# vbronetskyi/nclt-slam-project

Measured on AMD Instinct MI355X. Metric: relocalization frames/sec @640x480, 10k-landmark DB; Hamming-match HBM GB/s, higher is better.
Workload: dtype u8; 1 GPU; 640x480 BGR frames, 10000-record landmark DB (640000 descriptors, rows=fixed64), global relocalization tick per frame: ORB(500) + whole-DB mutual Hamming scan + top-25 PnP-RANSAC(200); frames resident in HBM, every frame's 96-byte result record written to pinned host memory by the tick's last kernel; distinct_frames=32, preroll_steps=20, streams=4, records=10000, descriptors=640000, parallelism=frames sharded across ranks, database replicated, no collective

## Files before the change

### nclt-slam-project_amd/csrc/reloc_match.hip

```cpp
#include <stdlib.h>
#include <type_traits>
#include <utility>

#include "reloc_internal.h"

typedef uint32_t u32;

__device__ __forceinline__ u32 bcnt_acc(u32 x, u32 acc)
{
    u32 r;
    asm("v_bcnt_u32_b32 %0, %1, %2" : "=v"(r) : "v"(x), "v"(acc));
    return r;
}
__device__ __forceinline__ u32 min_u16(u32 a, u32 b)
{
    u32 r;
    asm("v_min_u16 %0, %1, %2" : "=v"(r) : "v"(a), "v"(b));
    return r;
}
template <u32 IDX>
__device__ __forceinline__ u32 key_fma(u32 d, u32 c128)
{
    u32 r;
    asm("v_fmaak_f32 %0, %1, %2, %3" : "=v"(r) : "v"(d), "v"(c128), "n"(IDX));
    return r;
}
__device__ __forceinline__ u32 ham8(const u32 q[8], const uint4 a, const uint4 b, u32 init)
{
    u32 acc = init;
    acc = bcnt_acc(q[0] ^ a.x, acc);
    acc = bcnt_acc(q[1] ^ a.y, acc);
    acc = bcnt_acc(q[2] ^ a.z, acc);
    acc = bcnt_acc(q[3] ^ a.w, acc);
    acc = bcnt_acc(q[4] ^ b.x, acc);
    acc = bcnt_acc(q[5] ^ b.y, acc);
    acc = bcnt_acc(q[6] ^ b.z, acc);
    acc = bcnt_acc(q[7] ^ b.w, acc);
    return acc;
}

__device__ __forceinline__ void ham8x2(const u32 q0[8], const u32 q1[8], const uint4 a, const uint4 b, u32 init0, u32 init1,
                                       u32 &d0, u32 &d1)
{
    const u32 w[8] = {a.x, a.y, a.z, a.w, b.x, b.y, b.z, b.w};
    u32 acc0 = init0, acc1 = init1;
#pragma unroll
    for (int k = 0; k < 8; ++k) {
        const u32 x0 = q0[k] ^ w[k], x1 = q1[k] ^ w[k];
        acc0 = bcnt_acc(x0, acc0);
        acc1 = bcnt_acc(x1, acc1);
    }
    d0 = acc0;
    d1 = acc1;
}

template <int NC>
__device__ __forceinline__ void ham8_cols(const u32 (&q)[NC][8], const u32 (&w)[8], u32 (&h)[NC])
{
#pragma unroll
    for (int k = 0; k < 8; ++k)
#pragma unroll
        for (int j = 0; j < NC; ++j) {
            u32 x;
            asm volatile("v_xor_b32 %0, %1, %2" : "=v"(x) : "s"(w[k]), "v"(q[j][k]));
            if (k == 0) asm volatile("v_bcnt_u32_b32 %0, %1, 0" : "=v"(h[j]) : "v"(x));
            else asm volatile("v_bcnt_u32_b32 %0, %1, %0" : "+v"(h[j]) : "v"(x));
        }
}

__device__ __forceinline__ void srow_landed(u32 first_dword) { asm volatile("" ::"s"(first_dword)); }

__device__ __forceinline__ u32 umin(u32 a, u32 b) { return a < b ? a : b; }
__device__ __forceinline__ double uniform_f64(double v)
{
    return __hiloint2double(__builtin_amdgcn_readfirstlane(__double2hiint(v)), __builtin_amdgcn_readfirstlane(__double2loint(v)));
}
__device__ __forceinline__ u32 umax(u32 a, u32 b) { return a > b ? a : b; }

template <int K>
__device__ __forceinline__ u32 bfly(u32 a, u32 b, int lane)
{
    if constexpr (K == 32) {
        auto r = __builtin_amdgcn_permlane32_swap(a, b, false, false);
        return umin(r[0], r[1]);
    } else if constexpr (K == 16) {
        auto r = __builtin_amdgcn_permlane16_swap(a, b, false, false);
        return umin(r[0], r[1]);
    } else {
        const bool hi = lane & K;
        const u32 mine = hi ? b : a;
        const u32 theirs = hi ? a : b;
        return umin(mine, dpp_xor<K>(theirs));
    }
}

template <int K>
__device__ __forceinline__ u32 bfly_dpp(u32 a, u32 b)
{
    static_assert(K == 4 || K == 8, "bank-maskable lane bits only");
    u32 r;
    if constexpr (K == 4)
        asm("s_nop 1\n\tv_min_u32_dpp %0, %1, %1 row_shl:4 row_mask:0xf bank_mask:0x5\n\t"
            "v_min_u32_dpp %0, %2, %2 row_shr:4 row_mask:0xf bank_mask:0xa" : "=&v"(r) : "v"(a), "v"(b));
    else
        asm("s_nop 1\n\tv_min_u32_dpp %0, %1, %1 row_ror:8 row_mask:0xf bank_mask:0x3\n\t"
            "v_min_u32_dpp %0, %2, %2 row_ror:8 row_mask:0xf bank_mask:0xc" : "=&v"(r) : "v"(a), "v"(b));
    return r;
}
__device__ __forceinline__ u32 allmin_quad(u32 x)
{
    asm("s_nop 1\n\tv_min_u32_dpp %0, %0, %0 quad_perm:[1,0,3,2] row_mask:0xf bank_mask:0xf\n\t"
        "s_nop 1\n\tv_min_u32_dpp %0, %0, %0 quad_perm:[2,3,0,1] row_mask:0xf bank_mask:0xf" : "+v"(x));
    return x;
}

__device__ __forceinline__ u32 row_entry(u32 best, u32 lane)
{
    u32 v;
    asm("v_lshl_or_b32 %0, %1, 6, %2" : "=v"(v) : "v"(best), "v"(lane));
    return v;
}
__device__ __forceinline__ u32 row_key(u32 m, u32 colbase) { return ((m << 3) & 0xFFFF0000u) | ((m & 0x1FFu) | colbase); }
__device__ __forceinline__ u32 col_key(u32 k16, int tc)
{
    u32 key = k16 << 9;
    const u32 row = (k16 >> 3) & 15u;
    asm("v_add_u32_sdwa %0, %1, %2 dst_sel:WORD_0 dst_unused:UNUSED_PRESERVE src0_sel:DWORD src1_sel:DWORD"
        : "+v"(key) : "s"(tc), "v"(row));
    return key;
}

template <class F, int... I>
__device__ __forceinline__ void static_for_impl(F &&f, std::integer_sequence<int, I...>) { (f(std::integral_constant<int, I>{}), ...); }
template <int N, class F>
__device__ __forceinline__ void static_for(F &&f) { static_for_impl(f, std::make_integer_sequence<int, N>{}); }

template <int NJ>
__device__ __forceinline__ void scan_chunk(const uint4 *__restrict__ rec, int n, int tc, int nr, const u32 (&q)[NJ][8],
                                           u32 colbase, u32 *rowkey, u32 *colbest, bool single_cb, int lane)
{
    u32 cb16[NJ];
    const u32 c128 = 0x43000000u;
    constexpr int R = 16, LOG_R = 4;
    u32 stk[LOG_R + 1];
    auto bitrev = [](int i) { int r = 0; for (int b = 0; b < LOG_R; ++b) r |= ((i >> b) & 1) << (LOG_R - 1 - b); return r; };
    auto row_of = [&](int i) { return min(tc + bitrev(i), n - 1); };
    uint4 a = rec[2 * row_of(0)], b = rec[2 * row_of(0) + 1];
    static_for<R>([&](auto ic_) {
        constexpr int i = decltype(ic_)::value;
        constexpr int t = [](int v) { int r = 0; for (int bb = 0; bb < LOG_R; ++bb) r |= ((v >> bb) & 1) << (LOG_R - 1 - bb); return r; }(i);
        srow_landed(a.x);
        uint4 na, nb;
        if (i + 1 < R) { na = rec[2 * row_of(i + 1)]; nb = rec[2 * row_of(i + 1) + 1]; }
        __builtin_amdgcn_sched_barrier(0);
        u32 v = 0xFFFFFFFFu;
        if (t == 0 || t < nr) {
            u32 best = 0;
            const u32 w[8] = {a.x, a.y, a.z, a.w, b.x, b.y, b.z, b.w};
            u32 h[NJ];
            ham8_cols<NJ>(q, w, h);
            static_for<NJ / 2>([&](auto jc_) {
                constexpr int j = 2 * decltype(jc_)::value;
                const u32 k0 = key_fma<t * 8 + j>(h[j], c128), k1 = key_fma<t * 8 + j + 1>(h[j + 1], c128);
                cb16[j] = t == 0 ? k0 : min_u16(cb16[j], k0);
                cb16[j + 1] = t == 0 ? k1 : min_u16(cb16[j + 1], k1);
                best = j == 0 ? min_u16(k0, k1) : min_u16(best, min_u16(k0, k1));
            });
            v = row_entry(best, (u32)lane);
        }
        if constexpr ((i & 1) == 0) stk[0] = v;
        else {
            v = bfly_dpp<4>(stk[0], v);
            if constexpr ((i & 2) == 0) stk[1] = v;
            else {
                v = bfly_dpp<8>(stk[1], v);
                if constexpr ((i & 4) == 0) stk[2] = v;
                else {
                    v = bfly<16>(stk[2], v, lane);
                    if constexpr ((i & 8) == 0) stk[3] = v;
                    else stk[4] = bfly<32>(stk[3], v, lane);
                }
            }
        }
        __builtin_amdgcn_sched_barrier(0);
        if (i + 1 < R) { a = na; b = nb; }
    });
    const u32 m = allmin_quad(stk[LOG_R]);
    const int row_in_chunk = ((lane >> 2) & 1) * 8 + ((lane >> 3) & 1) * 4 + ((lane >> 4) & 1) * 2 + (lane >> 5);
    const bool writer = (lane & 3) == 0;
    const int row = tc + row_in_chunk;
    if (writer && row_in_chunk < nr) {
        if (single_cb) rowkey[row] = row_key(m, 0);
        else atomicMin(&rowkey[row], row_key(m, colbase));
    }
    u32 ck[NJ];
#pragma unroll
    for (int j = 0; j < NJ; ++j) ck[j] = col_key(cb16[j], tc);
    __builtin_amdgcn_sched_barrier(0);
#pragma unroll
    for (int j = 0; j < NJ; ++j) atomicMin(&colbest[colbase + j * 64 + lane], ck[j]);
}

struct WaveBinding {
    bool bound;
    int my_cb;
    int chunk0, chunk_step;
};
template <int NW>
__device__ __forceinline__ WaveBinding bind_wave(int wave, int ncb)
{
    const bool bound = (NW % ncb) == 0;
    return {bound, bound ? wave % ncb : 0, bound ? wave / ncb : wave, bound ? NW / ncb : NW};
}

template <int NJ, int NW>
__device__ __forceinline__ void db_emit_body(
    u32 *lds, int C, const uint4 *__restrict__ db, const int64_t *__restrict__ off, const int32_t *__restrict__ rec_ids,
    const int32_t *__restrict__ n_ids_p, int n_ids_max, const uint4 *__restrict__ cur, int max_rows,
    int32_t *__restrict__ m_qidx, int32_t *__restrict__ m_tidx, int32_t *__restrict__ m_dist, int32_t *__restrict__ m_n,
    int emit_stride, const float *__restrict__ g_pts3d, const float *__restrict__ g_xy, float *__restrict__ g_obj,
    float *__restrict__ g_img)
{
    constexpr int CB = 64 * NJ;
    const int tid = threadIdx.x, lane = tid & 63;
    const int wave = __builtin_amdgcn_readfirstlane(tid >> 6);
    const int n_ids = n_ids_p ? min(*n_ids_p, n_ids_max) : n_ids_max;
    const int ncb = max((C + CB - 1) / CB, 1);
    u32 *colbest = lds;
    u32 *rowkey = colbest + ncb * CB;
    u32 *wsum = rowkey + max_rows;
    static_assert(NW == 1 || NW == 2 || NW == 4 || NW == 8, "wsum holds one word per wave");

    u32 q[NJ][8];
    auto load_q = [&](int colbase) {
#pragma unroll
        for (int j = 0; j < NJ; ++j) {
            const int col = min(colbase + j * 64 + lane, max(C - 1, 0));
            const uint4 a = cur[2 * col], b = cur[2 * col + 1];
            q[j][0] = a.x; q[j][1] = a.y; q[j][2] = a.z; q[j][3] = a.w;
            q[j][4] = b.x; q[j][5] = b.y; q[j][6] = b.z; q[j][7] = b.w;
        }
    };
    const WaveBinding wb = bind_wave<NW>(wave, ncb);
    if (wb.bound) load_q(wb.my_cb * CB);
    for (int it = blockIdx.x; it < n_ids; it += gridDim.x) {
        const int r = rec_ids ? rec_ids[it] : it;
        const int64_t row0 = off[r];
        const int n = (int)(off[r + 1] - row0);
        const uint4 *rec = db + 2 * row0;
        for (int i = tid; i < ncb * CB; i += 64 * NW) colbest[i] = 0xFFFFFFFFu;
        for (int i = tid; i < n; i += 64 * NW) rowkey[i] = 0xFFFFFFFFu;
        __syncthreads();
        if (n > 0 && C > 0) {
            for (int cb = wb.bound ? wb.my_cb : 0; cb < (wb.bound ? wb.my_cb + 1 : ncb); ++cb) {
                if (!wb.bound) load_q(cb * CB);
                const int per = n / wb.chunk_step, extra = n % wb.chunk_step;
                int tc = wb.chunk0 * per + min(wb.chunk0, extra);
                const int tend = tc + per + (wb.chunk0 < extra ? 1 : 0);
#pragma nounroll
                for (; tc < tend; tc += 16)
                    scan_chunk<NJ>(rec, n, tc, min(16, tend - tc), q, (u32)(cb * CB), rowkey, colbest, ncb == 1, lane);
            }
        }
        __syncthreads();
        u32 base = 0;
        for (int rb = 0; rb < n; rb += 64 * NW) {
            const int row = rb + tid;
            bool mutual = false;
            u32 key = 0;
            if (row < n && C > 0) {
                key = rowkey[row];
                const u32 col = key & 0xFFFFu;
                mutual = (colbest[col] & 0xFFFFu) == (u32)row;
            }
            const unsigned long long bal = __ballot(mutual);
            if (lane == 0) wsum[wave] = (u32)__popcll(bal);
            __syncthreads();
            u32 before = base;
            for (int w = 0; w < wave; ++w) before += wsum[w];
            u32 total = 0;
            for (int w = 0; w < NW; ++w) total += wsum[w];
            if (mutual) {
                const u32 pos = before + (u32)__popcll(bal & ((1ull << lane) - 1ull));
                const int64_t o = (int64_t)it * emit_stride + pos;
                m_qidx[o] = row;
                m_tidx[o] = (int32_t)(key & 0xFFFFu);
                m_dist[o] = (int32_t)(key >> 16);
                if (g_obj) {
                    const float *p3 = g_pts3d + 3 * (row0 + row), *p2 = g_xy + 2 * (size_t)(key & 0xFFFFu);
                    float *po = g_obj + 3 * o, *pi = g_img + 2 * o;
                    po[0] = p3[0]; po[1] = p3[1]; po[2] = p3[2];
                    pi[0] = p2[0]; pi[1] = p2[1];
                }
            }
            base += total;
            __syncthreads();
        }
        if (tid == 0 && m_n) m_n[it] = (int32_t)base;
    }
}

constexpr int TICKET_STRIDE = 32;
constexpr int SCAN_TICKET_WORDS = (RELOC_BATCH_MAX * 8 + 1) * TICKET_STRIDE;
template <int NJ>
__device__ __forceinline__ void db_count_body(
    u32 *lds, int C, const uint4 *__restrict__ db, const int64_t *__restrict__ off, const int32_t *__restrict__ rec_ids,
    const int32_t *__restrict__ n_ids_p, int n_ids_max, const uint4 *__restrict__ cur, int max_rows,
    int32_t *__restrict__ counts, const ScanMask &mask, u32 *ticket, int quota, int n_bounded, int col_words,
    u32 *ticket_pool = nullptr, int pool_frames = 1, int block = -1, int n_blocks = -1)
{
    if (!ticket_pool) ticket_pool = ticket;
    if (block < 0) { block = blockIdx.x; n_blocks = gridDim.x; }
    constexpr int CB = 64 * NJ, NW = 4;
    const int tid = threadIdx.x, lane = tid & 63;
    const int wave = __builtin_amdgcn_readfirstlane(tid >> 6);
    const int n_ids = n_ids_p ? min(*n_ids_p, n_ids_max) : n_ids_max;
    const int ncb = max((C + CB - 1) / CB, 1);
    const bool dbl = 2 * ncb * CB <= col_words;
    u32 *colbuf = lds;
    u32 *rowkey = colbuf + col_words;
    u32 *wsum = rowkey + max_rows;

    u32 q[NJ][8];
    auto load_q = [&](int colbase) {
#pragma unroll
        for (int j = 0; j < NJ; ++j) {
            const int col = min(colbase + j * 64 + lane, max(C - 1, 0));
            const uint4 a = cur[2 * col], b = cur[2 * col + 1];
            q[j][0] = a.x; q[j][1] = a.y; q[j][2] = a.z; q[j][3] = a.w;
            q[j][4] = b.x; q[j][5] = b.y; q[j][6] = b.z; q[j][7] = b.w;
        }
    };
    const WaveBinding wb = bind_wave<NW>(wave, ncb);
    const bool stand_down = mask.skip_if && *mask.skip_if != 0;
    if (wb.bound && !stand_down) load_q(wb.my_cb * CB);
    double hc = 1.0, hs = 0.0, cos_tol = 0.0;
    if (mask.xyh) {
        cur_heading_q(mask.q, hc, hs);
        cos_tol = mask.cos_tol;
        hc = uniform_f64(hc); hs = uniform_f64(hs); cos_tol = uniform_f64(cos_tol);
    }
    int shard = 0, dry = 0;
    if (ticket) {
        u32 x;
        asm volatile("s_getreg_b32 %0, hwreg(HW_REG_XCC_ID, 0, 4)" : "=s"(x));
        shard = (int)(x & 7u);
    }
    auto draw = [&]() -> u32 { return atomicAdd(&ticket[shard * TICKET_STRIDE], 1u); };
    auto settle = [&](u32 t) -> int {
        for (;;) {
            const long long rec_i = (long long)n_blocks + (long long)shard + 8ll * (long long)t;
            if (rec_i < n_ids) return (int)rec_i;
            if (++dry >= 8) return n_ids;
            shard = (shard + 1) & 7;
            t = draw();
        }
    };
    int it = stand_down ? n_ids : block;
    int left = (quota > 0 && block < n_bounded) ? quota : 0x7fffffff;
    const bool dealer = tid == 64 * (NW - 1);
    const int buf_words = ncb * CB;
    for (int i = tid; i < buf_words; i += 64 * NW) colbuf[i] = 0xFFFFFFFFu;
    if (tid == 0) wsum[0] = wsum[1] = 0;
    __syncthreads();
    int p = 0;
    while (it < n_ids) {
        u32 *colbest = colbuf + (dbl ? p * buf_words : 0);
        const int r = rec_ids ? rec_ids[it] : it;
        const bool scored = !(mask.xyh && !heading_ok(mask.xyh + 4 * (int64_t)r, hc, hs, cos_tol));
        const int64_t row0 = off[r];
        const int n_rec = scored ? (int)(off[r + 1] - row0) : 0;
        const int n = C > 0 ? n_rec : 0;
        const uint4 *rec = db + 2 * row0;
        left -= max(n_rec, 1);
        u32 next_ticket = 0;
        if (ticket && dealer && left > 0) next_ticket = draw();
        if (n > 0) {
            if (ncb > 1) {
                for (int i = tid; i < n; i += 64 * NW) rowkey[i] = 0xFFFFFFFFu;
                __syncthreads();
            }
            for (int cb = wb.bound ? wb.my_cb : 0; cb < (wb.bound ? wb.my_cb + 1 : ncb); ++cb) {
                if (!wb.bound) load_q(cb * CB);
                const int per = n / wb.chunk_step, extra = n % wb.chunk_step;
                int tc = wb.chunk0 * per + min(wb.chunk0, extra);
                const int tend = tc + per + (wb.chunk0 < extra ? 1 : 0);
#pragma nounroll
                for (; tc < tend; tc += 16)
                    scan_chunk<NJ>(rec, n, tc, min(16, tend - tc), q, (u32)(cb * CB), rowkey, colbest, ncb == 1, lane);
            }
        }
        if (dbl) {
            u32 *other = colbuf + (p ^ 1) * buf_words;
            for (int base = 0; base + 128 * wave < buf_words; base += 128 * NW) {
                other[base + 2 * tid] = 0xFFFFFFFFu;
                other[base + 2 * tid + 1] = 0xFFFFFFFFu;
            }
        }
        __syncthreads();
        for (int rb = 0; rb + 64 * wave < n; rb += 64 * NW) {
            const int row = rb + tid;
            if (row < n) {
                const u32 col = rowkey[row] & 0xFFFFu;
                const unsigned long long mutual = __builtin_amdgcn_ballot_w64((colbest[col] & 0xFFFFu) == (u32)row);
                if (lane == 0 && mutual) atomicAdd(&wsum[p], (u32)__popcll(mutual));
            }
        }
        if (dealer) wsum[8] = ticket ? (left > 0 ? (u32)settle(next_ticket) : (u32)n_ids) : (u32)(it + n_blocks);
        __syncthreads();
        if (tid == 0) {
            counts[r] = (int32_t)wsum[p];
            wsum[p] = 0;
        }
        it = __builtin_amdgcn_readfirstlane((int)wsum[8]);
        if (dbl) p ^= 1;
        else {
            for (int i = tid; i < ncb * CB; i += 64 * NW) colbuf[i] = 0xFFFFFFFFu;
            __syncthreads();
        }
    }
    if (ticket && tid == 0) {
        const int words = pool_frames * 8;
        if (atomicAdd(&ticket_pool[words * TICKET_STRIDE], 1u) == gridDim.x - 1) {
            for (int x = 0; x <= words; ++x)
                __hip_atomic_store(&ticket_pool[x * TICKET_STRIDE], 0u, __ATOMIC_RELAXED, __HIP_MEMORY_SCOPE_AGENT);
        }
    }
}

template <int NJ>
__global__ __launch_bounds__(256, 4) RELOC_SCAN_VGPR_ATTR void k_db_scan(
    const uint4 *__restrict__ db, const int64_t *__restrict__ off, const int32_t *__restrict__ rec_ids,
    const int32_t *__restrict__ n_ids_p, int n_ids_max, const uint4 *__restrict__ cur,
    const int32_t *__restrict__ n_cur_p, int n_cur_max, int max_rows, int32_t *__restrict__ counts, ScanMask mask, u32 *ticket,
    int quota, int n_bounded, int col_words)
{
    extern __shared__ u32 lds[];
    const int C = n_cur_p ? min(*n_cur_p, n_cur_max) : n_cur_max;
    db_count_body<NJ>(lds, C, db, off, rec_ids, n_ids_p, n_ids_max, cur, max_rows, counts, mask, ticket, quota, n_bounded, col_words);
}

template <int NJ, int NW>
__global__ __launch_bounds__(64 * NW, 16 / NW) RELOC_SCAN_VGPR_ATTR void k_db_scan_emit(
    const uint4 *__restrict__ db, const int64_t *__restrict__ off, const int32_t *__restrict__ rec_ids,
    const int32_t *__restrict__ n_ids_p, int n_ids_max, const uint4 *__restrict__ cur,
    const int32_t *__restrict__ n_cur_p, int n_cur_max, int max_rows, int32_t *__restrict__ m_qidx,
    int32_t *__restrict__ m_tidx, int32_t *__restrict__ m_dist, int32_t *__restrict__ m_n, int emit_stride,
    const float *__restrict__ g_pts3d, const float *__restrict__ g_xy, float *__restrict__ g_obj, float *__restrict__ g_img)
{
    extern __shared__ u32 lds[];
    RELOC_SMALL_KERNEL_PRIO();
    const int C = n_cur_p ? min(*n_cur_p, n_cur_max) : n_cur_max;
    db_emit_body<NJ, NW>(lds, C, db, off, rec_ids, n_ids_p, n_ids_max, cur, max_rows, m_qidx, m_tidx, m_dist, m_n, emit_stride, g_pts3d,
                         g_xy, g_obj, g_img);
}

struct EmitFrame {
    const int32_t *rec_ids, *n_ids_p; const uint4 *cur; const int32_t *n_cur_p;
    int32_t *m_qidx, *m_tidx, *m_dist, *m_n; const float *g_xy; float *g_obj, *g_img;
};
struct EmitBatch { EmitFrame f[RELOC_BATCH_MAX]; };
static EmitFrame emit_frame(const reloc_ctx *c)
{
    EmitFrame F;
    const TickState &t = c->tick;
    const OrbFrame &o = c->orb.buf;
    F.rec_ids = t.cand_ids; F.n_ids_p = t.cand_n; F.cur = (const uint4 *)o.f_desc; F.n_cur_p = o.f_count;
    F.m_qidx = t.m_qidx; F.m_tidx = t.m_tidx; F.m_dist = t.m_dist; F.m_n = t.m_n; F.g_xy = o.f_xy; F.g_obj = t.p_obj; F.g_img = t.p_img;
    return F;
}

__global__ __launch_bounds__(256, 4) RELOC_SCAN_VGPR_ATTR void k_db_scan_emit_batch(const uint4 *__restrict__ db, const int64_t *__restrict__ off, int n_ids_max,
                                                          int n_cur_max, int max_rows, int emit_stride, const float *__restrict__ g_pts3d,
                                                          EmitBatch bt)
{
    extern __shared__ u32 lds[];
    RELOC_SMALL_KERNEL_PRIO();
    const EmitFrame &F = bt.f[blockIdx.y];
    const int C = F.n_cur_p ? min(*F.n_cur_p, n_cur_max) : n_cur_max;
    db_emit_body<8, 4>(lds, C, db, off, F.rec_ids, F.n_ids_p, n_ids_max, F.cur, max_rows, F.m_qidx, F.m_tidx, F.m_dist, F.m_n, emit_stride,
                       g_pts3d, F.g_xy, F.g_obj, F.g_img);
}

static int scan_lds_bytes(const char *who, int col_words, int max_rows, size_t &lds)
{
    lds = (size_t)(col_words + max_rows + 16) * 4;
    if (lds > 160 * 1024) { reloc_set_error("%s: LDS demand %zu bytes", who, lds); return RELOC_E_CAPACITY; }
    return RELOC_OK;
}

struct ScanBatch {
    int n;
    const uint4 *cur[RELOC_BATCH_MAX];
    const int32_t *n_cur[RELOC_BATCH_MAX];
    int32_t *counts[RELOC_BATCH_MAX];
    const int32_t *skip_if[RELOC_BATCH_MAX];
    double q[RELOC_BATCH_MAX][4];
    const double *xyh;
    double cos_tol;
};

__global__ __launch_bounds__(256, 4) RELOC_SCAN_VGPR_ATTR void k_db_scan_batch(const uint4 *__restrict__ db, const int64_t *__restrict__ off, int n_ids,
                                                          int n_cur_max, int max_rows, ScanBatch bt, u32 *ticket_pool, int quota, int n_bounded, int col_words)
{
    extern __shared__ u32 lds[];
    const int f = blockIdx.x % bt.n;
    ScanMask mask;
    mask.xyh = bt.xyh;
    for (int k = 0; k < 4; ++k) mask.q[k] = bt.q[f][k];
    mask.cos_tol = bt.cos_tol;
    mask.skip_if = bt.skip_if[f];
    const int C = bt.n_cur[f] ? min(*bt.n_cur[f], n_cur_max) : n_cur_max;
    db_count_body<8>(lds, C, db, off, nullptr, nullptr, n_ids, bt.cur[f], max_rows, bt.counts[f], mask, ticket_pool + f * 8 * TICKET_STRIDE, quota,
                     n_bounded, col_words, ticket_pool, bt.n, (int)(blockIdx.x / bt.n), (int)((gridDim.x + bt.n - 1 - f) / bt.n));
}

__device__ __forceinline__ u32 max_u16(u32 a, u32 b)
{
    u32 r;
    asm("v_max_u16 %0, %1, %2" : "=v"(r) : "v"(a), "v"(b));
    return r;
}

template <bool TICK>
__device__ __forceinline__ void db_ratio_body(const uint4 *__restrict__ db, const int64_t *__restrict__ off, int n_rec,
                                              const uint4 *__restrict__ cur, int C, double ratio, int32_t *__restrict__ counts,
                                              const ScanMask &mask, int min_rows, int block, int n_blocks)
{
    __shared__ u32 s_part[4][512];
    __shared__ int s_cnt[4];
    const int tid = threadIdx.x, lane = tid & 63;
    const int wave = __builtin_amdgcn_readfirstlane(tid >> 6);
    const int ncb = max((C + 511) >> 9, 1);
    double hc = 1.0, hs = 0.0, cos_tol = 0.0;
    if constexpr (TICK) {
        if (mask.skip_if && *mask.skip_if != 0) return;
        if (mask.xyh) {
            cur_heading_q(mask.q, hc, hs);
            hc = uniform_f64(hc); hs = uniform_f64(hs); cos_tol = uniform_f64(mask.cos_tol);
        }
    }
    u32 q[8][8];
    auto load_q = [&](int colbase) {
#pragma unroll
        for (int j = 0; j < 8; ++j) {
            const int col = min(colbase + j * 64 + lane, max(C - 1, 0));
            const uint4 a = cur[2 * col], b = cur[2 * col + 1];
            q[j][0] = a.x; q[j][1] = a.y; q[j][2] = a.z; q[j][3] = a.w;
            q[j][4] = b.x; q[j][5] = b.y; q[j][6] = b.z; q[j][7] = b.w;
        }
    };
    if (ncb == 1 && C > 0) load_q(0);
    for (int r = block; r < n_rec; r += n_blocks) {
        const int64_t row0 = off[r];
        int n = (int)(off[r + 1] - row0);
        if constexpr (TICK) {
            if (n < min_rows || (mask.xyh && !heading_ok(mask.xyh + 4 * (int64_t)r, hc, hs, cos_tol))) n = 0;
        }
        const uint4 *rec = db + 2 * row0;
        int good = 0;
        if (n >= 2 && C > 0) {
            for (int cb = 0; cb < ncb; ++cb) {
                if (ncb > 1) load_q(cb * 512);
                u32 k0[8], k1[8];
#pragma unroll
                for (int j = 0; j < 8; ++j) { k0[j] = 0xFFFFu; k1[j] = 0xFFFFu; }
                for (int t0 = wave * 8; t0 < n; t0 += 32) {
                    auto row_of = [&](int t) { return min(t0 + t, n - 1); };
                    uint4 a = rec[2 * row_of(0)], b = rec[2 * row_of(0) + 1];
#pragma unroll
                    for (int t = 0; t < 8; ++t) {
                        srow_landed(a.x);
                        uint4 na, nb;
                        if (t + 1 < 8) { na = rec[2 * row_of(t + 1)]; nb = rec[2 * row_of(t + 1) + 1]; }
                        __builtin_amdgcn_sched_barrier(0);
                        if (t0 + t < n) {
#pragma unroll
                            for (int j = 0; j < 8; j += 2) {
                                u32 h0, h1;
                                ham8x2(q[j], q[j + 1], a, b, 0, 0, h0, h1);
                                const u32 m0 = max_u16(k0[j], h0), m1 = max_u16(k0[j + 1], h1);
                                k0[j] = min_u16(k0[j], h0); k0[j + 1] = min_u16(k0[j + 1], h1);
                                k1[j] = min_u16(k1[j], m0); k1[j + 1] = min_u16(k1[j + 1], m1);
                            }
                        }
                        __builtin_amdgcn_sched_barrier(0);
                        if (t + 1 < 8) { a = na; b = nb; }
                    }
                }
#pragma unroll
                for (int j = 0; j < 8; ++j) s_part[wave][j * 64 + lane] = (k1[j] << 16) | k0[j];
                __syncthreads();
                for (int c = tid; c < 512; c += 256) {
                    u32 a0 = 0xFFFFu, a1 = 0xFFFFu;
                    for (int w = 0; w < 4; ++w) {
                        const u32 v = s_part[w][c];
                        const u32 lo = v & 0xFFFFu, hi = v >> 16;
                        const u32 n0 = a0 < lo ? a0 : lo;
                        const u32 n1 = a0 < lo ? (a1 < lo ? a1 : lo) : (hi < a0 ? hi : a0);
                        a0 = n0; a1 = n1;
                    }
                    const bool ok = cb * 512 + c < C && a1 != 0xFFFFu && (double)a0 < ratio * (double)a1;
                    good += __popcll(__ballot(ok));
                }
                __syncthreads();
            }
        }
        if (lane == 0) s_cnt[wave] = good;
        __syncthreads();
        if (tid == 0) counts[r] = s_cnt[0] + s_cnt[1] + s_cnt[2] + s_cnt[3];
        __syncthreads();
    }
}

template <bool TICK>
__global__ __launch_bounds__(256, 4) void k_db_ratio(const uint4 *__restrict__ db, const int64_t *__restrict__ off, int n_rec,
                                                     const uint4 *__restrict__ cur, const int32_t *__restrict__ n_cur_p,
                                                     int n_cur_max, double ratio, int32_t *__restrict__ counts, ScanMask mask,
                                                     int min_rows)
{
    const int C = n_cur_p ? min(*n_cur_p, n_cur_max) : n_cur_max;
    db_ratio_body<TICK>(db, off, n_rec, cur, C, ratio, counts, mask, min_rows, blockIdx.x, gridDim.x);
}

__global__ __launch_bounds__(256, 4) void k_db_ratio_batch(const uint4 *__restrict__ db, const int64_t *__restrict__ off, int n_rec,
                                                           int n_cur_max, double ratio, ScanBatch bt, int min_rows)
{
    const int f = blockIdx.y;
    ScanMask mask;
    mask.xyh = bt.xyh;
    for (int k = 0; k < 4; ++k) mask.q[k] = bt.q[f][k];
    mask.cos_tol = bt.cos_tol;
    mask.skip_if = bt.skip_if[f];
    const int C = bt.n_cur[f] ? min(*bt.n_cur[f], n_cur_max) : n_cur_max;
    db_ratio_body<true>(db, off, n_rec, bt.cur[f], C, ratio, bt.counts[f], mask, min_rows, blockIdx.x, gridDim.x);
}

constexpr int RATIO_KEY_SHIFT = 22;
template <int NW>
// ... 182 lines not shown
                     "v_permlane16_swap_b32 %0, %4\n\t"
                     "v_permlane16_swap_b32 %8, %12\n\t"
                     "v_min_u16 %0, %0, %4\n\t"
                     "v_min_u16 %8, %8, %12\n\t"
                     SQ_NOP
                     "v_permlane32_swap_b32 %0, %8\n\t"
                     "v_min_u16 %0, %0, %8\n\t"
                     SQ_NOP SQ_Q1("%0") SQ_NOP SQ_Q2("%0")
                     : "+v"(d[0]), "+v"(d[1]), "+v"(d[2]), "+v"(d[3]), "+v"(d[4]), "+v"(d[5]), "+v"(d[6]), "+v"(d[7]), "+v"(d[8]),
                       "+v"(d[9]), "+v"(d[10]), "+v"(d[11]), "+v"(d[12]), "+v"(d[13]), "+v"(d[14]), "+v"(d[15]));
    } else if constexpr (G == 8) {
        asm volatile(SQ_NOP
                     SQ_N4("%0", "%1") SQ_N4("%2", "%3") SQ_N4("%4", "%5") SQ_N4("%6", "%7")
                     SQ_N8("%0", "%2") SQ_N8("%4", "%6")
                     SQ_NOP
                     "v_permlane16_swap_b32 %0, %4\n\t"
                     "v_min_u16 %0, %0, %4\n\t"
                     SQ_NOP SQ_Q1("%0") SQ_NOP SQ_Q2("%0")
                     "v_mov_b32 %4, %0\n\t"
                     SQ_NOP
                     "v_permlane32_swap_b32 %0, %4\n\t"
                     "v_min_u16 %0, %0, %4\n\t"
                     : "+v"(d[0]), "+v"(d[1]), "+v"(d[2]), "+v"(d[3]), "+v"(d[4]), "+v"(d[5]), "+v"(d[6]), "+v"(d[7]));
    } else {
        static_assert(G == 4, "groups of 4, 8 or 16 queries");
        asm volatile(SQ_NOP
                     SQ_N4("%0", "%1") SQ_N4("%2", "%3")
                     SQ_NOP
                     SQ_N8("%0", "%2")
                     SQ_NOP SQ_Q1("%0") SQ_NOP SQ_Q2("%0")
                     "v_mov_b32 %2, %0\n\t"
                     SQ_NOP
                     "v_permlane16_swap_b32 %0, %2\n\t"
                     "v_min_u16 %0, %0, %2\n\t"
                     "v_mov_b32 %2, %0\n\t"
                     SQ_NOP
                     "v_permlane32_swap_b32 %0, %2\n\t"
                     "v_min_u16 %0, %0, %2\n\t"
                     : "+v"(d[0]), "+v"(d[1]), "+v"(d[2]), "+v"(d[3]));
    }
    return d[0];
}
#undef SQ_N4
#undef SQ_N8
#undef SQ_Q1
#undef SQ_Q2
#undef SQ_NOP
template <int G>
__device__ __forceinline__ u32 sq_lane_of(u32 q)
{
    if constexpr (G == 16) return ((q & 15u) << 2) | (q >> 4);
    else if constexpr (G == 8) return ((q & 7u) << 2) | ((q >> 3) & 3u) | (q & 32u);
    else return (q & 3u) << 2;
}

template <int G, bool HOIST>
__global__ __launch_bounds__(64 * SQ_WAVES) __attribute__((amdgpu_waves_per_eu(8, 8))) void k_db_scan_rows(
    const uint4 *__restrict__ db, const int64_t *__restrict__ off, int n_rec, const uint4 *__restrict__ cur,
    const int32_t *__restrict__ n_cur_p, int n_cur_max, int32_t *__restrict__ counts)
{
    __shared__ unsigned short s_row[SQ_WAVES][SQ_MAX_ROWS];
    const int lane = threadIdx.x & 63;
    const int wave = __builtin_amdgcn_readfirstlane((int)(threadIdx.x >> 6));
    const int C = n_cur_p ? min(*n_cur_p, n_cur_max) : n_cur_max;
    unsigned short *rowk = s_row[wave];
    const int gw = blockIdx.x * SQ_WAVES + wave, nw = gridDim.x * SQ_WAVES;
    const int my_group = G == 16 ? (lane & 3) : (G == 8 ? ((lane & 3) | ((lane >> 5) << 2)) : 0);
    constexpr int NH = HOIST ? G : 1;
    u32 qs[NH][8];
    if constexpr (HOIST) {
#pragma unroll
        for (int j = 0; j < G; ++j) {
            const int q = max(min(j, C - 1), 0);
            const uint4 qa = cur[2 * q], qb = cur[2 * q + 1];
            qs[j][0] = qa.x; qs[j][1] = qa.y; qs[j][2] = qa.z; qs[j][3] = qa.w;
            qs[j][4] = qb.x; qs[j][5] = qb.y; qs[j][6] = qb.z; qs[j][7] = qb.w;
        }
    }
    auto chunk = [&](const uint4 a, const uint4 b, int tc, u32 &colk) -> u32 {
        const u32 w[8] = {a.x, a.y, a.z, a.w, b.x, b.y, b.z, b.w};
        u32 rbest = 0xFFFFu;
        for (int q0 = 0; q0 < (HOIST ? 1 : C); q0 += G) {
            u32 ck[G];
#pragma unroll
            for (int j4 = 0; j4 < G; j4 += 4) {
                u32 hs[4];
                if constexpr (HOIST) {
                    const u32 (&qv)[4][8] = *reinterpret_cast<const u32 (*)[4][8]>(&qs[j4 < NH ? j4 : 0]);
                    sq_dist4(qv, w, hs);
                } else {
                    u32 qw[4][8];
                    sq_load4(cur, q0 + j4, C, qw);
                    sq_dist4(qw, w, hs);
                }
#pragma unroll
                for (int jj = 0; jj < 4; ++jj) {
                    rbest = min_u16(rbest, hs[jj] | (u32)(q0 + j4 + jj));
                    ck[j4 + jj] = hs[jj] | (u32)lane;
                }
            }
            const u32 m = sq_bfly<G>(ck);
            const u32 key = ((m >> 6) << 16) | (u32)(tc + (int)(m & 63u));
            const u32 better = umin(colk, key);
            colk = my_group * G == q0 ? better : colk;
        }
        return rbest;
    };
    for (int r = gw; r < n_rec; r += nw) {
        const int64_t row0 = off[r];
        const int n = (int)(off[r + 1] - row0);
        if (n <= 0 || C <= 0) {
            if (lane == 0) counts[r] = 0;
            continue;
        }
        const uint4 *rec = db + 2 * row0;
        u32 colk = 0xFFFFFFFFu;
        int total;
        {
            const int row = min(lane, n - 1);
            const u32 rb = chunk(rec[2 * row], rec[2 * row + 1], 0, colk);
            if (n <= 64) {
                const u32 peer = (u32)__builtin_amdgcn_ds_bpermute((int)(sq_lane_of<G>(rb & 63u) << 2), (int)colk);
                total = __popcll(__ballot(lane < n && (peer & 0xFFFFu) == (u32)lane));
                if (lane == 0) counts[r] = total;
                continue;
            }
            rowk[lane] = (unsigned short)rb;
        }
        for (int tc = 64; tc < n; tc += 64) {
            const int row = min(tc + lane, n - 1);
            const u32 rb = chunk(rec[2 * row], rec[2 * row + 1], tc, colk);
            if (tc + lane < n) rowk[tc + lane] = (unsigned short)rb;
        }
        total = 0;
        for (int tc = 0; tc < n; tc += 64) {
            const u32 k = tc + lane < n ? rowk[tc + lane] : 0u;
            const u32 peer = (u32)__builtin_amdgcn_ds_bpermute((int)(sq_lane_of<G>(k & 63u) << 2), (int)colk);
            total += __popcll(__ballot(tc + lane < n && (peer & 0xFFFFu) == (u32)(tc + lane)));
        }
        if (lane == 0) counts[r] = total;
    }
}

struct CountPlan {
    int col_words = 0;
    size_t lds = 0;
    int resident = 0;
    int quota = 0, n_bounded = 0;

    int init(const reloc_ctx *ctx, const char *who, int nj, int n_cur_max, int max_rows)
    {
        const int cb = 64 * nj, ncb = (n_cur_max + cb - 1) / cb;
        col_words = (ncb >= 2 ? ncb : 2) * cb;
        if (int rc = scan_lds_bytes(who, col_words, max_rows, lds)) return rc;
        const int wg_per_cu = (int)(160 * 1024 / lds);
        resident = ctx->num_cu * (wg_per_cu < 4 ? wg_per_cu : 4);
        return RELOC_OK;
    }

    void budget(const reloc_ctx *ctx, int workgroups)
    {
        const DbArena &db = ctx_db(ctx);
        const int n_ids = (int)db.records;
        if (workgroups > n_ids) workgroups = n_ids;
        if (workgroups < 1) workgroups = 1;
        const int q_rec = (n_ids + workgroups - 1) / workgroups;
        n_bounded = (n_ids + q_rec - 1) / q_rec;
        quota = (int)((db.rows * q_rec + n_ids - 1) / n_ids);
        if (quota < 1) quota = 1;
    }
};

int scan_alloc(reloc_ctx *ctx)
{
    if (int rc = ctx_dev_alloc(ctx, &ctx->scan_ticket, SCAN_TICKET_WORDS)) return rc;
    HIP_TRY(hipMemset(ctx->scan_ticket, 0, SCAN_TICKET_WORDS * sizeof(uint32_t)));
    return RELOC_OK;
}

int launch_db_count(reloc_ctx *ctx, const uint8_t *cur, const int32_t *n_cur_dev, int n_cur_max, int32_t *counts, const ScanMask &mask)
{
    const DbArena &db = ctx_db(ctx);
    const int n_ids = (int)db.records;
    if (n_ids <= 0) return RELOC_OK;
    if (n_cur_max > 65535) { reloc_set_error("db scan: more than 65535 current descriptors"); return RELOC_E_CAPACITY; }
    if (db.max_rows > MAX_REC_ROWS) { reloc_set_error("db scan: record larger than %d rows", MAX_REC_ROWS); return RELOC_E_CAPACITY; }
    const int max_rows = db.max_rows < 1 ? 1 : db.max_rows;
    const uint4 *desc = (const uint4 *)db.desc;
    if (!mask.xyh && n_cur_max <= 64 && max_rows <= SQ_MAX_ROWS) {
        if (n_cur_max == 0) {
            HIP_TRY(hipMemsetAsync(counts, 0, (size_t)n_ids * sizeof(int32_t), ctx->stream));
            return RELOC_OK;
        }
        int grid = ctx->num_cu * 8;
        const int need = (n_ids + SQ_WAVES - 1) / SQ_WAVES;
        if (grid > need) grid = need;
#define RELOC_LAUNCH_ROWS(G, HOIST)                                                                                           \
    hipLaunchKernelGGL((k_db_scan_rows<G, HOIST>), dim3(grid), dim3(64 * SQ_WAVES), 0, ctx->stream, desc, db.off, n_ids, \
                       (const uint4 *)cur, n_cur_dev, n_cur_max, counts)
        if (n_cur_max <= 4) RELOC_LAUNCH_ROWS(4, true); else if (n_cur_max <= 8) RELOC_LAUNCH_ROWS(8, false); else RELOC_LAUNCH_ROWS(16, false);
#undef RELOC_LAUNCH_ROWS
        HIP_TRY(hipGetLastError());
        return RELOC_OK;
    }
    const int nj = n_cur_max <= 128 ? 2 : (n_cur_max <= 256 ? 4 : 8);
    CountPlan p;
    if (int rc = p.init(ctx, "db scan", nj, n_cur_max, max_rows)) return rc;
    int grid = ctx->num_cu * 16;
    u32 *ticket = nullptr;
    if (nj == 8 && n_ids > p.resident && ctx->scan_ticket) {
        ticket = ctx->scan_ticket;
        grid = p.resident;
        if (ctx->scan_gens > 0) {
            p.budget(ctx, p.resident * ctx->scan_gens);
            grid = p.n_bounded + 8;
        }
    }
    if (grid > n_ids) grid = n_ids;
#define RELOC_LAUNCH_COUNT(NJ)                                                                                               \
    hipLaunchKernelGGL((k_db_scan<NJ>), dim3(grid), dim3(256), p.lds, ctx->stream, desc, db.off, nullptr, nullptr, n_ids,       \
                       (const uint4 *)cur, n_cur_dev, n_cur_max, max_rows, counts, mask, ticket, p.quota, p.n_bounded, p.col_words)
    if (nj == 2) RELOC_LAUNCH_COUNT(2); else if (nj == 4) RELOC_LAUNCH_COUNT(4); else RELOC_LAUNCH_COUNT(8);
#undef RELOC_LAUNCH_COUNT
    HIP_TRY(hipGetLastError());
    return RELOC_OK;
}

static int launch_db_emit(reloc_ctx *const *ctxs, int n, const EmitBatch &bt, const uint8_t *db_desc, const int64_t *db_off,
                          int max_rows, const float *g_pts3d, int n_ids_max, int n_cur_max, int emit_stride, bool latency)
{
    reloc_ctx *c0 = ctxs[0];
    if (n < 1 || n > RELOC_BATCH_MAX) { reloc_set_error("emit: 1..%d frames", RELOC_BATCH_MAX); return RELOC_E_ARG; }
    if (n_ids_max <= 0) return RELOC_OK;
    if (n_cur_max > 65535) { reloc_set_error("db scan: more than 65535 current descriptors"); return RELOC_E_CAPACITY; }
    if (max_rows > MAX_REC_ROWS) { reloc_set_error("db scan: record larger than %d rows", MAX_REC_ROWS); return RELOC_E_CAPACITY; }
    if (max_rows < 1) max_rows = 1;
    const int nj = n > 1 || n_cur_max > 256 ? 8 : (n_cur_max <= 128 ? 2 : 4);
    const int cb = 64 * nj;
    const int ncb = (n_cur_max + cb - 1) / cb > 0 ? (n_cur_max + cb - 1) / cb : 1;
    size_t lds;
    if (int rc = scan_lds_bytes("db scan", ncb * cb, max_rows, lds)) return rc;
    const int grid = n_ids_max < c0->num_cu * 16 ? n_ids_max : c0->num_cu * 16;
    if (n == 1) {
        const EmitFrame &F = bt.f[0];
#define RELOC_LAUNCH_EMIT(NJ, NW)                                                                                            \
    hipLaunchKernelGGL((k_db_scan_emit<NJ, NW>), dim3(grid), dim3(64 * NW), lds, c0->stream, (const uint4 *)db_desc, db_off, F.rec_ids, \
                       F.n_ids_p, n_ids_max, F.cur, F.n_cur_p, n_cur_max, max_rows, F.m_qidx, F.m_tidx, F.m_dist, F.m_n, emit_stride, \
                       g_pts3d, F.g_xy, F.g_obj, F.g_img)
        if (latency) {
            if (nj == 2) RELOC_LAUNCH_EMIT(2, 8); else if (nj == 4) RELOC_LAUNCH_EMIT(4, 8); else RELOC_LAUNCH_EMIT(8, 8);
        } else {
            if (nj == 2) RELOC_LAUNCH_EMIT(2, 4); else if (nj == 4) RELOC_LAUNCH_EMIT(4, 4); else RELOC_LAUNCH_EMIT(8, 4);
        }
#undef RELOC_LAUNCH_EMIT
    } else {
        hipLaunchKernelGGL(k_db_scan_emit_batch, dim3(grid, n), dim3(256), lds, c0->stream, (const uint4 *)db_desc, db_off, n_ids_max,
                           n_cur_max, max_rows, emit_stride, g_pts3d, bt);
    }
    HIP_TRY(hipGetLastError());
    return RELOC_OK;
}

static int launch_db_ratio_emit(reloc_ctx *const *ctxs, int n, const EmitBatch &bt, const uint8_t *db_desc, const int64_t *db_off,
                                const float *g_pts3d, int n_ids_max, int n_cur_max, int emit_stride, double ratio, int min_rows,
                                int gate_off, bool latency)
{
    reloc_ctx *c0 = ctxs[0];
    if (n < 1 || n > RELOC_BATCH_MAX) { reloc_set_error("emit: 1..%d frames", RELOC_BATCH_MAX); return RELOC_E_ARG; }
    if (n_ids_max <= 0) return RELOC_OK;
    if (n_cur_max > 65535) { reloc_set_error("db scan: more than 65535 current descriptors"); return RELOC_E_CAPACITY; }
    if (n_cur_max > emit_stride) {
        reloc_set_error("ratio match lists: %d current descriptors do not fit the list stride of %d", n_cur_max, emit_stride);
        return RELOC_E_CAPACITY;
    }
    const int grid = n_ids_max < c0->num_cu * 16 ? n_ids_max : c0->num_cu * 16;
    const uint4 *desc = (const uint4 *)db_desc;
    if (n > 1)
        hipLaunchKernelGGL(k_db_ratio_emit_batch, dim3(grid, n), dim3(256), 0, c0->stream, desc, db_off, n_ids_max, n_cur_max, ratio,
                           min_rows, gate_off, emit_stride, g_pts3d, bt);
    else if (latency)
        hipLaunchKernelGGL(k_db_ratio_emit<8>, dim3(grid), dim3(512), 0, c0->stream, desc, db_off, n_ids_max, n_cur_max, ratio,
                           min_rows, gate_off, emit_stride, g_pts3d, bt.f[0]);
    else
        hipLaunchKernelGGL(k_db_ratio_emit<4>, dim3(grid), dim3(256), 0, c0->stream, desc, db_off, n_ids_max, n_cur_max, ratio,
                           min_rows, gate_off, emit_stride, g_pts3d, bt.f[0]);
    HIP_TRY(hipGetLastError());
    return RELOC_OK;
}

int launch_tick_emit(reloc_ctx *const *ctxs, int n, bool latency)
{
    reloc_ctx *c0 = ctxs[0];
    const DbArena &db = ctx_db(c0);
    EmitBatch bt;
    frame_slots(ctxs, n, [&](int f, reloc_ctx *c, int) { bt.f[f] = emit_frame(c); });
    if (c0->match.ratio_on())
        return launch_db_ratio_emit(ctxs, n, bt, db.desc, db.off, db.pts3d, MAX_CAND, c0->max_feat, MAX_REC_ROWS, c0->match.ratio,
                                    c0->prm.min_matches, MAX_CAND, latency);
    return launch_db_emit(ctxs, n, bt, db.desc, db.off, db.max_rows, db.pts3d, MAX_CAND, c0->max_feat, MAX_REC_ROWS, latency);
}

int launch_db_scan_batch(reloc_ctx *const *ctxs, int n, const double *q, double cos_tol, bool auto_mode, bool heading_mask)
{
    reloc_ctx *c0 = ctxs[0];
    if (n < 1 || n > RELOC_BATCH_MAX) { reloc_set_error("scan batch: 1..%d frames", RELOC_BATCH_MAX); return RELOC_E_ARG; }
    const DbArena &db = ctx_db(c0);
    if (c0->max_feat > 65535 || db.max_rows > MAX_REC_ROWS) { reloc_set_error("scan batch: capacity"); return RELOC_E_CAPACITY; }
// ... 381 lines not shown
```

Baseline: 7570 frames/s.

## Merge column minima via per-wave LDS slices for small records instead of atomics

For records with at most 64 rows under a single column block, each wave writes its 16-bit column minima into a private LDS slice rather than doing atomicMin into a shared column buffer. After the barrier, one thread per row combines the four wave slices to check mutual matches, and the column-buffer reset and double-buffer flip are skipped on that path. The aim is to remove LDS atomic traffic and the buffer-clearing work for small records. In exchange it adds LDS space for the slices, which can lower workgroups per CU, and it branches on an opaque copy of n. An uninitialised-register trick also drops the 0xFFFFFFFF initialisation of row entries.

```diff
diff --git a/nclt-slam-project_amd/csrc/reloc_match.hip b/nclt-slam-project_amd/csrc/reloc_match.hip
--- a/nclt-slam-project_amd/csrc/reloc_match.hip
+++ b/nclt-slam-project_amd/csrc/reloc_match.hip
@@ -135,9 +135,11 @@
 template <int N, class F>
 __device__ __forceinline__ void static_for(F &&f) { static_for_impl(f, std::make_integer_sequence<int, N>{}); }
 
-template <int NJ>
+enum ScanMerge { MERGE_SHARED, MERGE_CHOICE };
+template <int NJ, ScanMerge MERGE = MERGE_SHARED>
 __device__ __forceinline__ void scan_chunk(const uint4 *__restrict__ rec, int n, int tc, int nr, const u32 (&q)[NJ][8],
-                                           u32 colbase, u32 *rowkey, u32 *colbest, bool single_cb, int lane)
+                                           u32 colbase, u32 *rowkey, u32 *colbest, bool single_cb, int lane,
+                                           unsigned short *slice = nullptr, int sliced_max = -1)
 {
     u32 cb16[NJ];
     const u32 c128 = 0x43000000u;
@@ -153,7 +155,8 @@
         uint4 na, nb;
         if (i + 1 < R) { na = rec[2 * row_of(i + 1)]; nb = rec[2 * row_of(i + 1) + 1]; }
         __builtin_amdgcn_sched_barrier(0);
-        u32 v = 0xFFFFFFFFu;
+        u32 v;
+        asm("" : "=v"(v));
         if (t == 0 || t < nr) {
             u32 best = 0;
             const u32 w[8] = {a.x, a.y, a.z, a.w, b.x, b.y, b.z, b.w};
@@ -192,6 +195,13 @@
     if (writer && row_in_chunk < nr) {
         if (single_cb) rowkey[row] = row_key(m, 0);
         else atomicMin(&rowkey[row], row_key(m, colbase));
+    }
+    if constexpr (MERGE == MERGE_CHOICE) {
+        if (n <= sliced_max) {
+#pragma unroll
+            for (int j = 0; j < NJ; ++j) slice[j * 64 + lane] = (unsigned short)cb16[j];
+            return;
+        }
     }
     u32 ck[NJ];
 #pragma unroll
@@ -320,6 +330,7 @@
     u32 *colbuf = lds;
     u32 *rowkey = colbuf + col_words;
     u32 *wsum = rowkey + max_rows;
+    unsigned short *slices = (unsigned short *)(wsum + 16);
 
     u32 q[NJ][8];
     auto load_q = [&](int colbase) {
@@ -364,6 +375,7 @@
     if (tid == 0) wsum[0] = wsum[1] = 0;
     __syncthreads();
     int p = 0;
+    const int sliced_max = ncb == 1 ? 16 * NW : -1;
     while (it < n_ids) {
         u32 *colbest = colbuf + (dbl ? p * buf_words : 0);
         const int r = rec_ids ? rec_ids[it] : it;
@@ -375,6 +387,7 @@
         left -= max(n_rec, 1);
         u32 next_ticket = 0;
         if (ticket && dealer && left > 0) next_ticket = draw();
+        auto sliced = [&]() { int nn = n; asm volatile("" : "+s"(nn)); return nn <= sliced_max; };
         if (n > 0) {
             if (ncb > 1) {
                 for (int i = tid; i < n; i += 64 * NW) rowkey[i] = 0xFFFFFFFFu;
@@ -387,17 +400,40 @@
                 const int tend = tc + per + (wb.chunk0 < extra ? 1 : 0);
 #pragma nounroll
                 for (; tc < tend; tc += 16)
-                    scan_chunk<NJ>(rec, n, tc, min(16, tend - tc), q, (u32)(cb * CB), rowkey, colbest, ncb == 1, lane);
+                    scan_chunk<NJ, MERGE_CHOICE>(rec, n, tc, min(16, tend - tc), q, (u32)(cb * CB), rowkey, colbest, ncb == 1, lane,
+                                                 slices + wave * CB, sliced_max);
             }
         }
-        if (dbl) {
-            u32 *other = colbuf + (p ^ 1) * buf_words;
-            for (int base = 0; base + 128 * wave < buf_words; base += 128 * NW) {
-                other[base + 2 * tid] = 0xFFFFFFFFu;
-                other[base + 2 * tid + 1] = 0xFFFFFFFFu;
+        if (!sliced()) {
+            asm volatile("");
+            if (dbl) {
+                u32 *other = colbuf + (p ^ 1) * buf_words;
+                for (int base = 0; base + 128 * wave < buf_words; base += 128 * NW) {
+                    other[base + 2 * tid] = 0xFFFFFFFFu;
+                    other[base + 2 * tid + 1] = 0xFFFFFFFFu;
+                }
             }
         }
         __syncthreads();
+        if (sliced()) {
+            if (64 * wave < n) {
+                asm volatile("");
+                if (tid < n) {
+                    const u32 col = rowkey[tid] & 0xFFFFu;
+                    const int per = n / NW, extra = n % NW;
+                    u32 best = 0xFFFFFFFFu;
+#pragma unroll
+                    for (int w = 0; w < NW; ++w)
+                        if (w < n) {
+                            const u32 k = slices[w * CB + col];
+                            const u32 tc_w = (u32)(w * per + min(w, extra));
+                            best = umin(best, ((k << 9) & 0xFFFF0000u) | (tc_w + ((k >> 3) & 15u)));
+                        }
+                    const unsigned long long mutual = __builtin_amdgcn_ballot_w64((best & 0xFFFFu) == (u32)tid);
+                    if (lane == 0 && mutual) atomicAdd(&wsum[p], (u32)__popcll(mutual));
+                }
+            }
+        } else
         for (int rb = 0; rb + 64 * wave < n; rb += 64 * NW) {
             const int row = rb + tid;
             if (row < n) {
@@ -413,6 +449,7 @@
             wsum[p] = 0;
         }
         it = __builtin_amdgcn_readfirstlane((int)wsum[8]);
+        if (sliced()) continue;
         if (dbl) p ^= 1;
         else {
             for (int i = tid; i < ncb * CB; i += 64 * NW) colbuf[i] = 0xFFFFFFFFu;
@@ -482,9 +519,9 @@
                        g_pts3d, F.g_xy, F.g_obj, F.g_img);
 }
 
-static int scan_lds_bytes(const char *who, int col_words, int max_rows, size_t &lds)
-{
-    lds = (size_t)(col_words + max_rows + 16) * 4;
+static int scan_lds_bytes(const char *who, int col_words, int max_rows, size_t &lds, int slice_keys = 0)
+{
+    lds = (size_t)(col_words + max_rows + 16) * 4 + (size_t)slice_keys * 2;
     if (lds > 160 * 1024) { reloc_set_error("%s: LDS demand %zu bytes", who, lds); return RELOC_E_CAPACITY; }
     return RELOC_OK;
 }
@@ -973,7 +1010,7 @@
     {
         const int cb = 64 * nj, ncb = (n_cur_max + cb - 1) / cb;
         col_words = (ncb >= 2 ? ncb : 2) * cb;
-        if (int rc = scan_lds_bytes(who, col_words, max_rows, lds)) return rc;
+        if (int rc = scan_lds_bytes(who, col_words, max_rows, lds, 4 * cb)) return rc;
         const int wg_per_cu = (int)(160 * 1024 / lds);
         resident = ctx->num_cu * (wg_per_cu < 4 ? wg_per_cu : 4);
         return RELOC_OK;
```

Result: faster. 7651 frames/s, median of 6 (+1.1%).
